# BLu85/AES-GCM-128-192-256-bits

Measured on NVIDIA B200. Metric: aes_gcm_enc_tag_throughput, higher is better.
Workload: dtype u8

## Files before the change

aes-gcm-128-192-256-bits_b200/csrc/capi.cu:

```cuda
#include <cuda.h>
#include <cuda_runtime.h>
#include <stdint.h>
#include <stdio.h>
#include <stdlib.h>
#include <string.h>
#include <new>
#include <vector>

#include "../../include/aesgcm_b200.h"
#include "kernels.h"
#include "host_sched.h"

namespace {

constexpr int kSlots = 3;
constexpr size_t kChunkBytesMax = 64u << 20;
constexpr size_t kMaxChunks = 8192;
constexpr uint64_t kAadInlineMax = 4096;
constexpr uint64_t kMaxBlocks = 0xFFFFFFFEull;

constexpr size_t SC_PART_CT = 0;
constexpr size_t SC_TAGCALC = 32;
constexpr size_t SC_OK = 48;
constexpr size_t SC_TAG = 64;
constexpr size_t SC_J0 = 80;
constexpr size_t SC_KEY = 96;
constexpr size_t SC_PARTS = 256;
constexpr size_t SC_PARTS_MAX = 1024;
constexpr size_t SC_BYTES = SC_PARTS + 16 * (SC_PARTS_MAX + 1);

template <class T>
struct GrownBuf {
    T* p = nullptr;
    size_t cap = 0;
};

struct PowCache {
    uint32_t* d = nullptr;
    uint64_t e = ~0ull;
    cudaEvent_t ev = nullptr;
    cudaStream_t st = nullptr;
};

}

struct agcm_ctx {
    int device = 0, sm_count = 0, ncta = 0, nt = 0;
    uint32_t* d_te0 = nullptr;
    KeyDev* d_key = nullptr;
    uint32_t* d_parts = nullptr;
    GrownBuf<uint32_t> seg_parts;
    uint8_t* d_scratch = nullptr;
    uint32_t* d_counters = nullptr;
    PowCache pow_n;
    PowCache pow_scale;
    uint32_t j0ctr = 1;
    GrownBuf<uint8_t> iv_stage;
    uint8_t** d_peer_bufs = nullptr;
    uint32_t* d_peer_status = nullptr;
    uint32_t* h_peer_status = nullptr;
    int peer_rank = 0, peer_world = 0;
    uint32_t peer_epoch = 0;
    uint64_t peer_timeout_ns = 10000000000ull;
    cudaStream_t peer_side = nullptr;
    cudaEvent_t peer_bulk_ev[AG_PEER_RING] = {};
    cudaEvent_t peer_fin_ev[AG_PEER_RING] = {};
    uint32_t h_rk[60];
    uint8_t h_H[16];
    uint8_t h_key_in[240];
    size_t key_in_len = 0;
    int key_in_mode = 0, key_in_pre = 0;
    int nr = 0;
    bool key_set = false;
    cudaError_t last_err = cudaSuccess;
    uint64_t launches = 0;
    bool timing = false;
    static constexpr int kTimingRing = 64;
    cudaEvent_t tev[2 * kTimingRing] = {};
    int tev_pending = 0;
    double t_total_ms = 0.0;
    uint64_t t_count = 0;
    cudaStream_t hs[kSlots] = {nullptr, nullptr, nullptr};
    uint8_t* d_stage[kSlots] = {nullptr, nullptr, nullptr};
    uint8_t* d_stage_aux[kSlots] = {nullptr, nullptr, nullptr};
    uint32_t* d_stage_parts[kSlots] = {nullptr, nullptr, nullptr};
    uint8_t* d_chunk_partials = nullptr;
    GrownBuf<uint8_t> aad_stage;
    uint32_t* d_tile_ticket = nullptr;
    bool no_ticket = false;
    GrownBuf<uint32_t> sort;
    void* tmap_encode = nullptr;
    GrownBuf<uint8_t> verify;
    bool pipeline_ready = false;
    size_t chunk_bytes = 32u << 20;
    size_t ramp_base = 1u << 20;
};

namespace {

int cuda_fail(agcm_ctx* c, cudaError_t e)
{
    if (c) c->last_err = e;
    return AGCM_E_CUDA;
}

#define AG_CUDA(ctx, call)                              \
    do {                                                \
        cudaError_t _e = (call);                        \
// ... 13 lines not shown
void iv_words(const uint8_t iv[12], uint32_t w[3])
{
    for (int i = 0; i < 3; ++i)
        w[i] = (uint32_t)iv[4 * i] | ((uint32_t)iv[4 * i + 1] << 8) | ((uint32_t)iv[4 * i + 2] << 16) |
               ((uint32_t)iv[4 * i + 3] << 24);
}

int timing_drain(agcm_ctx* c)
{
    for (int i = 0; i < c->tev_pending; ++i) {
        AG_CUDA(c, cudaEventSynchronize(c->tev[2 * i + 1]));
        float ms = 0.f;
        AG_CUDA(c, cudaEventElapsedTime(&ms, c->tev[2 * i], c->tev[2 * i + 1]));
        c->t_total_ms += ms;
        c->t_count++;
    }
    c->tev_pending = 0;
    return AGCM_OK;
}

template <class T>
int grow(agcm_ctx* c, GrownBuf<T>& b, size_t need)
{
    if (need <= b.cap) return AGCM_OK;
    AG_CUDA(c, cudaFree(b.p));
    b.p = nullptr;
    b.cap = 0;
    AG_CUDA(c, cudaMalloc(&b.p, need));
    b.cap = need;
    return AGCM_OK;
}

int zeroed_ticket(agcm_ctx* c, size_t words, cudaStream_t st, uint32_t*& ticket)
{
    if (!c->d_tile_ticket) AG_CUDA(c, cudaMalloc(&c->d_tile_ticket, 4 * sizeof(uint32_t)));
    AG_CUDA(c, cudaMemsetAsync(c->d_tile_ticket, 0, words * sizeof(uint32_t), st));
    ticket = c->d_tile_ticket;
    return AGCM_OK;
}

int pow_get(agcm_ctx* c, PowCache& pc, uint64_t e, cudaStream_t st)
{
    if (pc.ev && pc.st != st) AG_CUDA(c, cudaStreamWaitEvent(st, pc.ev, 0));
    if (pc.e == e) return AGCM_OK;
    AG_CUDA(c, ag_launch_pow(c->d_key, e, pc.d, st));
    c->launches++;
    pc.e = e;
    if (!pc.ev) AG_CUDA(c, cudaEventCreateWithFlags(&pc.ev, cudaEventDisableTiming));
    AG_CUDA(c, cudaEventRecord(pc.ev, st));
    pc.st = st;
    return AGCM_OK;
}

int peer_join_stream(agcm_ctx* c, cudaStream_t st)
{
    if (c->peer_epoch && c->peer_fin_ev[0]) AG_CUDA(c, cudaStreamWaitEvent(st, c->peer_fin_ev[c->peer_epoch % AG_PEER_RING], 0));
    return AGCM_OK;
}

int ensure_pow(agcm_ctx* c, uint64_t n_blocks, cudaStream_t st)
{
    if (c->pow_n.e != n_blocks) {
        int rc = peer_join_stream(c, st);
        if (rc) return rc;
    }
    return pow_get(c, c->pow_n, n_blocks, st);
}

FinishParams finish_params(const agcm_ctx* c, int decrypt, const uint8_t iv[12], const uint8_t* d_aad, uint64_t aad_len,
                           uint64_t ct_len, uint8_t* d_tag, uint8_t* d_ok, const uint32_t* hn)
{
    FinishParams f;
    memset(&f, 0, sizeof(f));
    memcpy(f.rk, c->h_rk, sizeof(f.rk));
    f.nr = (uint32_t)c->nr;
    iv_words(iv, f.iv);
    f.j0w = __builtin_bswap32(c->j0ctr);
    f.key = c->d_key;
    f.te0 = c->d_te0;
    f.aad = d_aad;
    f.aad_len = aad_len;
    f.ct_len = ct_len;
    f.tag_calc = decrypt ? c->d_scratch + SC_TAGCALC : d_tag;
    f.tag_expected = decrypt ? d_tag : nullptr;
    f.ok = decrypt ? d_ok : nullptr;
    f.hn = hn;
    return f;
}

int run_stream(agcm_ctx* c, int mode, const uint8_t iv[12], uint64_t first_block, const uint8_t* d_in, uint8_t* d_out,
               uint64_t n_bytes, uint64_t blocks_after, uint32_t* parts_raw, uint8_t* d_partial16, cudaStream_t st,
               uint32_t* counter, const FinishParams* ff = nullptr, uint32_t peer_epoch = 0, const uint8_t* gate = nullptr)
{
    if (n_bytes == 0) {
        if (d_partial16) AG_CUDA(c, cudaMemsetAsync(d_partial16, 0, 16, st));
        return AGCM_OK;
    }
    StreamParams p;
    memset(&p, 0, sizeof(p));
    memcpy(p.rk, c->h_rk, sizeof(p.rk));
    iv_words(iv, p.iv);
    p.ctr0 = (uint32_t)(c->j0ctr + 1 + first_block);
    p.j0w = __builtin_bswap32(c->j0ctr);
    p.n_bytes = n_bytes;
    p.in = d_in;
    p.out = d_out;
    p.key = c->d_key;
    p.te0 = c->d_te0;
    p.partials = parts_raw;
    p.gate = gate;
    if (mode != AG_MODE_CTR_ONLY) {
        p.done_counter = counter;
        p.scale_e = blocks_after;
        if (blocks_after && counter == c->d_counters && mode != AG_MODE_GHASH_ONLY) {
            if (!c->pow_scale.d) AG_CUDA(c, cudaMalloc(&c->pow_scale.d, 16));
            int rc = pow_get(c, c->pow_scale, blocks_after, st);
            if (rc) return rc;
            p.scale_pow = c->pow_scale.d;
        }
        p.out16 = d_partial16;
        if (ff) {
            p.fuse_finish = 1;
            p.aad = ff->aad;
            p.aad_len = ff->aad_len;
            p.ct_len = ff->ct_len;
            p.tag_calc = ff->tag_calc;
            p.tag_expected = ff->tag_expected;
            p.ok = ff->ok;
            p.hn = ff->hn;
        }
        if (peer_epoch) {
            p.peer_bufs = c->d_peer_bufs;
            p.peer_rank = (uint32_t)c->peer_rank;
            p.peer_world = (uint32_t)c->peer_world;
            p.peer_epoch = peer_epoch;
        }
    }
    cudaEvent_t ev0 = nullptr, ev1 = nullptr;
    if (c->timing) {
        if (c->tev_pending == agcm_ctx::kTimingRing) {
            int rc = timing_drain(c);
            if (rc) return rc;
        }
        ev0 = c->tev[2 * c->tev_pending];
        ev1 = c->tev[2 * c->tev_pending + 1];
        AG_CUDA(c, cudaEventRecord(ev0, st));
    }
    int ncta = c->ncta;
    const uint64_t blocks = (n_bytes + 15) >> 4;
    if (blocks <= (uint64_t)c->ncta * (uint64_t)c->nt) ncta = (int)((blocks + (uint64_t)c->nt - 1) / (uint64_t)c->nt);
    AG_CUDA(c, ag_launch_stream(p, c->nr, mode, ncta, c->nt, st));
    c->launches++;
    if (c->timing) {
        AG_CUDA(c, cudaEventRecord(ev1, st));
        c->tev_pending++;
    }
    return AGCM_OK;
}

int run_finish(agcm_ctx* c, int decrypt, const uint8_t iv[12], const uint8_t* d_parts16, int n_parts, const uint8_t* d_aad,
               uint64_t aad_len, uint64_t ct_len, uint8_t* d_tag, uint8_t* d_ok, cudaStream_t st)
{
    if (n_parts < 0 || (size_t)n_parts > SC_PARTS_MAX) return AGCM_E_BAD_ARG;
    if (decrypt && (!d_tag || !d_ok)) return AGCM_E_BAD_ARG;
    if (!decrypt && !d_tag) return AGCM_E_BAD_ARG;
    const uint64_t n_ct_blocks = (ct_len + 15) >> 4;
    if (n_ct_blocks > kMaxBlocks) return AGCM_E_COUNTER_OVERFLOW;
    const uint8_t* parts = d_parts16;
    int np = n_parts;
    const uint8_t* aad_inline = (aad_len && d_aad) ? d_aad : nullptr;
    if (aad_len && !d_aad) return AGCM_E_BAD_ARG;
    if (aad_len > kAadInlineMax) {
        uint8_t* list = c->d_scratch + SC_PARTS;
        if (n_parts) AG_CUDA(c, cudaMemcpyAsync(list, d_parts16, 16 * (size_t)n_parts, cudaMemcpyDeviceToDevice, st));
        int rc = run_stream(c, AG_MODE_GHASH_ONLY, iv, 0, d_aad, nullptr, aad_len, n_ct_blocks,
                            c->d_parts + 4 * AG_MAX_CTA, list + 16 * (size_t)n_parts, st, c->d_counters);
        if (rc) return rc;
        parts = list;
        np = n_parts + 1;
        aad_inline = nullptr;
    }
    if (aad_inline) {
        int rc = ensure_pow(c, n_ct_blocks, st);
        if (rc) return rc;
    }
    FinishParams f = finish_params(c, decrypt, iv, aad_inline, aad_len, ct_len, d_tag, d_ok, aad_inline ? c->pow_n.d : nullptr);
    f.parts = parts;
    f.n_parts = (uint32_t)np;
    AG_CUDA(c, ag_launch_finish(f, st));
    c->launches++;
    return AGCM_OK;
}

int derive_j0(agcm_ctx* c, const uint8_t* h_iv, size_t iv_len, uint8_t j0[16], cudaStream_t st)
{
    if (!h_iv || iv_len == 0 || iv_len > (1ull << 32)) return AGCM_E_BAD_LEN;
    if (!c->key_set) return AGCM_E_NO_KEY;
    const size_t padded = ((iv_len + 15) & ~(size_t)15) + 16;
    std::vector<uint8_t> buf(padded, 0);
    memcpy(buf.data(), h_iv, iv_len);
    const uint64_t bits = (uint64_t)iv_len * 8;
    for (int i = 0; i < 8; ++i) buf[padded - 1 - i] = (uint8_t)(bits >> (8 * i));
    int rc = grow(c, c->iv_stage, padded < 4096 ? 4096 : padded);
    if (rc) return rc;
    AG_CUDA(c, cudaMemcpyAsync(c->iv_stage.p, buf.data(), padded, cudaMemcpyHostToDevice, st));
    const uint8_t iv0[12] = {0};
    rc = run_stream(c, AG_MODE_GHASH_ONLY, iv0, 0, c->iv_stage.p, nullptr, padded, 0, c->d_parts, c->d_scratch + SC_J0, st,
                    c->d_counters);
// ... 172 lines not shown
    }
    if (e != cudaSuccess) {
        agcm_ctx_destroy(c);
        return AGCM_E_CUDA;
    }
    *out = c;
    return AGCM_OK;
}

int agcm_ctx_create(agcm_ctx** out, int device) { return agcm_ctx_create_ex(out, device, 0, 0); }

void agcm_ctx_destroy(agcm_ctx* c)
{
    if (!c) return;
    cudaSetDevice(c->device);
    cudaDeviceSynchronize();
    for (int s = 0; s < kSlots; ++s) {
        if (c->hs[s]) cudaStreamDestroy(c->hs[s]);
        cudaFree(c->d_stage[s]);
        cudaFree(c->d_stage_aux[s]);
        cudaFree(c->d_stage_parts[s]);
    }
    for (cudaEvent_t e : c->tev)
        if (e) cudaEventDestroy(e);
    if (c->d_key) cudaMemset(c->d_key, 0, sizeof(KeyDev));
    if (c->d_scratch) cudaMemset(c->d_scratch, 0, SC_BYTES);
    memset(c->h_rk, 0, sizeof(c->h_rk));
    memset(c->h_H, 0, sizeof(c->h_H));
    memset(c->h_key_in, 0, sizeof(c->h_key_in));
    cudaFree(c->d_chunk_partials);
    cudaFree(c->aad_stage.p);
    cudaFree(c->verify.p);
    cudaFree(c->d_tile_ticket);
    cudaFree(c->sort.p);
    cudaFree(c->d_te0);
    cudaFree(c->d_key);
    cudaFree(c->d_parts);
    cudaFree(c->seg_parts.p);
    cudaFree(c->iv_stage.p);
    cudaFree(c->d_scratch);
    cudaFree(c->d_counters);
    cudaFree(c->pow_n.d);
    cudaFree(c->pow_scale.d);
    cudaFree(c->d_peer_bufs);
    cudaFree(c->d_peer_status);
    if (c->h_peer_status) cudaFreeHost(c->h_peer_status);
    if (c->peer_side) cudaStreamDestroy(c->peer_side);
    for (uint32_t i = 0; i < AG_PEER_RING; ++i) {
        if (c->peer_bulk_ev[i]) cudaEventDestroy(c->peer_bulk_ev[i]);
        if (c->peer_fin_ev[i]) cudaEventDestroy(c->peer_fin_ev[i]);
    }
    if (c->pow_n.ev) cudaEventDestroy(c->pow_n.ev);
    if (c->pow_scale.ev) cudaEventDestroy(c->pow_scale.ev);
    delete c;
}

int agcm_last_cuda_error(const agcm_ctx* c) { return c ? (int)c->last_err : 0; }
const char* agcm_last_cuda_error_string(const agcm_ctx* c) { return cudaGetErrorString(c ? c->last_err : cudaSuccess); }
uint64_t agcm_launch_count(const agcm_ctx* c) { return c ? c->launches : 0; }

int agcm_timing_enable(agcm_ctx* c, int on)
{
    if (!c) return AGCM_E_BAD_ARG;
    AG_CUDA(c, cudaSetDevice(c->device));
    if (on && !c->tev[0])
        for (cudaEvent_t& e : c->tev) AG_CUDA(c, cudaEventCreate(&e));
    int rc = timing_drain(c);
    if (rc) return rc;
    c->timing = on != 0;
    c->t_total_ms = 0.0;
    c->t_count = 0;
    return AGCM_OK;
}

int agcm_timing_read(agcm_ctx* c, double* total_ms, uint64_t* n_launches)
{
    if (!c) return AGCM_E_BAD_ARG;
    int rc = timing_drain(c);
    if (rc) return rc;
    if (total_ms) *total_ms = c->t_total_ms;
    if (n_launches) *n_launches = c->t_count;
    return AGCM_OK;
}

int agcm_get_info(const agcm_ctx* c, int* n_cta, int* threads, int* sm_count)
{
    if (!c) return AGCM_E_BAD_ARG;
    if (n_cta) *n_cta = c->ncta;
    if (threads) *threads = c->nt;
    if (sm_count) *sm_count = c->sm_count;
    return AGCM_OK;
}

int agcm_key_expand(agcm_ctx* c, int mode, const uint8_t* d_keys, size_t n_keys, uint8_t* d_round_keys, void* stream)
{
    if (!c || (n_keys && (!d_keys || !d_round_keys))) return AGCM_E_BAD_ARG;
    if (!mode_to_nr(mode)) return AGCM_E_BAD_MODE;
    AG_CUDA(c, cudaSetDevice(c->device));
    AG_CUDA(c, ag_launch_key_expand(d_keys, n_keys, mode / 8, c->d_te0, d_round_keys, (cudaStream_t)stream));
    if (n_keys) c->launches++;
    return AGCM_OK;
}

int agcm_key_expand_host(agcm_ctx* c, int mode, const uint8_t* h_key, uint8_t* h_round_keys)
{
    if (!c || !h_key || !h_round_keys) return AGCM_E_BAD_ARG;
    const int nr = mode_to_nr(mode);
    if (!nr) return AGCM_E_BAD_MODE;
    AG_CUDA(c, cudaSetDevice(c->device));
    uint8_t* d_key = c->d_scratch + SC_KEY;
    uint8_t* d_rk = c->d_scratch + SC_PARTS;
    AG_CUDA(c, cudaMemcpy(d_key, h_key, (size_t)mode / 8, cudaMemcpyHostToDevice));
    AG_CUDA(c, ag_launch_key_expand(d_key, 1, mode / 8, c->d_te0, d_rk, nullptr));
    c->launches++;
    AG_CUDA(c, cudaMemcpy(h_round_keys, d_rk, (size_t)16 * (nr + 1), cudaMemcpyDeviceToHost));
    return AGCM_OK;
}

int agcm_set_key(agcm_ctx* c, int mode, int pre_expanded, const uint8_t* h_key, size_t key_len)
{
    if (!c || !h_key) return AGCM_E_BAD_ARG;
    const int nr = mode_to_nr(mode);
    if (!nr) return AGCM_E_BAD_MODE;
    const size_t want = pre_expanded ? (size_t)16 * (nr + 1) : (size_t)mode / 8;
    if (key_len != want) return AGCM_E_BAD_MODE;
    if (c->key_set && c->key_in_mode == mode && c->key_in_pre == (pre_expanded ? 1 : 0) && c->key_in_len == key_len &&
        memcmp(c->h_key_in, h_key, key_len) == 0)
        return AGCM_OK;
    AG_CUDA(c, cudaSetDevice(c->device));
    c->key_set = false;
    c->pow_n.e = ~0ull;
    c->pow_scale.e = ~0ull;
    KeyIn in;
    memset(&in, 0, sizeof(in));
    memcpy(in.w, h_key, key_len);
    in.key_bytes = (uint32_t)mode / 8;
    in.nr = (uint32_t)nr;
    in.pre_expanded = pre_expanded ? 1u : 0u;
    AG_CUDA(c, cudaDeviceSynchronize());
    AG_CUDA(c, ag_launch_key_setup(c->d_key, in, c->d_te0, c->nt, c->ncta, nullptr));
    c->launches++;
    static_assert(offsetof(KeyDev, rk) == 0 && offsetof(KeyDev, H) == 256, "KeyDev head layout");
    uint32_t head[68];
    AG_CUDA(c, cudaMemcpy(head, c->d_key, sizeof(head), cudaMemcpyDeviceToHost));
    memset(c->h_rk, 0, sizeof(c->h_rk));
    memcpy(c->h_rk, head, (size_t)16 * (nr + 1));
    const uint32_t* hw = head + 64;
    for (int i = 0; i < 4; ++i) {
        c->h_H[4 * i + 0] = (uint8_t)(hw[i] >> 24);
        c->h_H[4 * i + 1] = (uint8_t)(hw[i] >> 16);
        c->h_H[4 * i + 2] = (uint8_t)(hw[i] >> 8);
        c->h_H[4 * i + 3] = (uint8_t)hw[i];
    }
    c->nr = nr;
    memcpy(c->h_key_in, h_key, key_len);
    c->key_in_len = key_len;
    c->key_in_mode = mode;
    c->key_in_pre = pre_expanded ? 1 : 0;
    c->key_set = true;
    return AGCM_OK;
}

int agcm_get_round_keys(const agcm_ctx* c, uint8_t* h_round_keys, size_t cap)
{
    if (!c || !h_round_keys) return AGCM_E_BAD_ARG;
    if (!c->key_set) return AGCM_E_NO_KEY;
    const size_t n = (size_t)16 * (c->nr + 1);
    if (cap < n) return AGCM_E_BAD_LEN;
    memcpy(h_round_keys, c->h_rk, n);
    return (int)n;
}

int agcm_get_h(const agcm_ctx* c, uint8_t h_h16[16])
{
    if (!c || !h_h16) return AGCM_E_BAD_ARG;
    if (!c->key_set) return AGCM_E_NO_KEY;
    memcpy(h_h16, c->h_H, 16);
    return AGCM_OK;
}

int agcm_stream_part(agcm_ctx* c, int decrypt, const uint8_t h_iv12[12], uint64_t first_block, const uint8_t* d_in,
                     uint8_t* d_out, uint64_t n_bytes, uint64_t blocks_after, uint8_t* d_partial16, void* stream)
{
    if (!c || !h_iv12 || !d_partial16 || (n_bytes && (!d_in || !d_out))) return AGCM_E_BAD_ARG;
    if (!c->key_set) return AGCM_E_NO_KEY;
// ... 1133 lines not shown
```

aes-gcm-128-192-256-bits_b200/csrc/gcm_core.cuh:

```cuda
#pragma once
#include <stdint.h>
#include <string.h>
#include "aes_core.cuh"
#include "gf128.cuh"

enum : int {
    AG_MODE_ENC = 0,
    AG_MODE_DEC = 1,
    AG_MODE_GHASH_ONLY = 2,
    AG_MODE_CTR_ONLY = 3
};

constexpr int AG_MAX_CTA = 256;
#ifndef AG_NT_MAX
#define AG_NT_MAX 512
#endif
constexpr int AG_STREAM_NT_MAX = AG_NT_MAX;

struct KeyDev {
    uint32_t rk[60];
    uint32_t nr;
    uint32_t nt_stream;
    uint32_t ncta;
    uint32_t _pad;
    gf128 H;
    gf128 pow2[64];
    gf128 hpow_thread[AG_STREAM_NT_MAX + 1];
    gf128 hpow_cta[AG_MAX_CTA + 1];
    uint4 tab[8][256];
};

AG_HD void ag_load_block(const uint8_t* p, uint32_t nvalid, uint32_t x[4])
{
    if (nvalid == 16) {
#if defined(__CUDA_ARCH__)
        const uintptr_t a = (uintptr_t)p;
        if ((a & 15) == 0) {
            const uint4 v = *reinterpret_cast<const uint4*>(p);
            x[0] = v.x; x[1] = v.y; x[2] = v.z; x[3] = v.w;
            return;
        }
        if ((a & 3) == 0) {
            const uint32_t* q = reinterpret_cast<const uint32_t*>(p);
            x[0] = q[0]; x[1] = q[1]; x[2] = q[2]; x[3] = q[3];
            return;
        }
#endif
    }
    x[0] = x[1] = x[2] = x[3] = 0;
#pragma unroll
    for (uint32_t j = 0; j < 16; ++j)
        if (j < nvalid) x[j >> 2] |= (uint32_t)p[j] << (8 * (j & 3));
}

AG_HD void ag_store_block(uint8_t* p, uint32_t nvalid, const uint32_t x[4])
// ... 123 lines not shown
    bool have;
    __device__ __forceinline__ void init() { have = false; prev_addr = nullptr; prev = make_uint4(0, 0, 0, 0); }
    __device__ __forceinline__ void flush()
    {
        if (!have) return;
        const uint32_t ro = (uint32_t)((uintptr_t)prev_addr & 15);
        const uint32_t w[4] = {prev.x, prev.y, prev.z, prev.w};
        uint8_t* q = prev_addr + 16 - ro;
        for (uint32_t j = 16 - ro; j < 16; ++j) q[j - (16 - ro)] = (uint8_t)(w[j >> 2] >> (8 * (j & 3)));
        have = false;
    }
    __device__ __forceinline__ void put(uint8_t* q, const uint32_t o[4])
    {
        const uint32_t ro = (uint32_t)((uintptr_t)q & 15);
        const uint4 cur = make_uint4(o[0], o[1], o[2], o[3]);
        if (have && prev_addr + 16 == q) {
            *reinterpret_cast<uint4*>(q - ro) = ag_realign(prev, cur, 16 - ro);
        } else {
            flush();
            for (uint32_t j = 0; j < 16 - ro; ++j) q[j] = (uint8_t)(o[j >> 2] >> (8 * (j & 3)));
        }
        prev = cur;
        prev_addr = q;
        have = true;
    }
};
#endif

struct StreamParams {
    uint32_t rk[60];
    uint32_t iv[3];
    uint32_t ctr0;
    uint32_t j0w;
    uint64_t n_bytes;
    const uint8_t* in;
    uint8_t* out;
    const KeyDev* key;
    const uint32_t* te0;
    uint32_t* partials;
    uint32_t* done_counter;
    uint64_t scale_e;
    const uint32_t* scale_pow;
    uint8_t* out16;
    uint32_t fuse_finish;
    const uint8_t* aad;
    uint64_t aad_len, ct_len;
    uint8_t* tag_calc;
    const uint8_t* tag_expected;
    uint8_t* ok;
    const uint32_t* hn;
    uint8_t* const* peer_bufs;
    uint32_t peer_rank, peer_world, peer_epoch;
    const uint8_t* gate;
};

constexpr uint32_t AG_PEER_MAX = 16;
constexpr uint32_t AG_PEER_RING = 8;
constexpr uint32_t AG_PEER_AHEAD = 4;
constexpr uint32_t AG_PEER_FLAGS = AG_PEER_RING * AG_PEER_MAX * 16;
constexpr uint32_t AG_PEER_BYTES = AG_PEER_FLAGS + AG_PEER_RING * AG_PEER_MAX * 4;

#if defined(__CUDA_ARCH__)
__device__ __forceinline__ void ag_store_row_coop(uint8_t* dst, const uint32_t o[4], bool whole, uint32_t r)
{
    const uint32_t lane = threadIdx.x & 31;
    uint4 prev;
    prev.x = __shfl_up_sync(0xffffffffu, o[0], 1);
    prev.y = __shfl_up_sync(0xffffffffu, o[1], 1);
    prev.z = __shfl_up_sync(0xffffffffu, o[2], 1);
    prev.w = __shfl_up_sync(0xffffffffu, o[3], 1);
    const bool prev_whole = __shfl_up_sync(0xffffffffu, (int)whole, 1) != 0 && lane > 0;
    const bool next_whole = __shfl_down_sync(0xffffffffu, (int)whole, 1) != 0 && lane < 31;
    if (!whole) return;
    if (prev_whole) {
        *reinterpret_cast<uint4*>(dst - r) = ag_realign(prev, make_uint4(o[0], o[1], o[2], o[3]), 16 - r);
    } else {
        ag_store_block(dst, 16 - r, o);
    }
    if (!next_whole) {
        const uint4 t = ag_realign(make_uint4(o[0], o[1], o[2], o[3]), make_uint4(0, 0, 0, 0), 16 - r);
        const uint32_t tw[4] = {t.x, t.y, t.z, t.w};
        ag_store_block(dst + 16 - r, r, tw);
    }
}
#endif

template <int NR, int MODE, bool ALIGNED, class TE, class GH>
AG_HD gf128 ag_stream_lane(const StreamParams& p, uint32_t g, uint32_t Gt, TE&& te, GH&& gh)
{
    const uint32_t n_blocks = (uint32_t)((p.n_bytes + 15) >> 4);
    const uint32_t n_full = (uint32_t)(p.n_bytes >> 4);
    const uint32_t rows = (uint32_t)(((uint64_t)n_blocks + Gt - 1) / Gt);
    const uint32_t pad = (uint32_t)((uint64_t)rows * Gt - n_blocks);
    const uint32_t tail = (uint32_t)(p.n_bytes & 15);

    AesCtrConst cc;
    AesCtrCache cache;
    bool have = rows && g >= pad;
    uint32_t i = g - pad;
    if (MODE != AG_MODE_GHASH_ONLY) {
        cc = aes_ctr_precompute(p.rk, p.iv[0], p.iv[1], p.iv[2], te);
        aes_ctr_cache_fill(p.rk, cc, ag_bswap32(p.ctr0 + i) ^ p.rk[3], te, cache);
    }

    auto load = [&](uint32_t bi, uint32_t x[4]) {
        const uint8_t* src = p.in + 16 * (uint64_t)bi;
        if (ALIGNED && bi < n_full) {
#if defined(__CUDA_ARCH__)
            const uint4 v = *reinterpret_cast<const uint4*>(src);
            x[0] = v.x; x[1] = v.y; x[2] = v.z; x[3] = v.w;
#else
            ag_load_block(src, 16, x);
#endif
        } else {
            ag_load_block_in(src, bi < n_full ? 16u : tail, x, p.in, p.in + p.n_bytes);
        }
    };

    gf128 y = gf_zero();
    uint32_t xn[4] = {0, 0, 0, 0};
#if defined(__CUDA_ARCH__)
    const uint32_t r_out = (uint32_t)((uintptr_t)p.out & 15);
    const bool coop = !ALIGNED && MODE != AG_MODE_GHASH_ONLY && (r_out & 3) != 0;
#endif
    if (have) load(i, xn);
    for (uint32_t u = 0; u < rows; ++u) {
        uint32_t x[4] = {xn[0], xn[1], xn[2], xn[3]};
        if (u + 1 < rows) load(i + Gt, xn);
        if (MODE != AG_MODE_CTR_ONLY && u) y = gf_mul_table(y, gh);
        uint32_t o[4] = {0, 0, 0, 0};
        bool whole_out = false;
        if (have) {
            uint32_t s[4];
            if (MODE == AG_MODE_GHASH_ONLY) {
                s[0] = x[0]; s[1] = x[1]; s[2] = x[2]; s[3] = x[3];
            } else {
                uint32_t ks[4];
                aes_ctr_block_cached<NR>(p.rk, cc, cache, p.ctr0 + i, te, ks);
                o[0] = x[0] ^ ks[0]; o[1] = x[1] ^ ks[1]; o[2] = x[2] ^ ks[2]; o[3] = x[3] ^ ks[3];
                uint8_t* dst = p.out + 16 * (uint64_t)i;
                if (ALIGNED && i < n_full) {
#if defined(__CUDA_ARCH__)
                    *reinterpret_cast<uint4*>(dst) = make_uint4(o[0], o[1], o[2], o[3]);
#else
                    ag_store_block(dst, 16, o);
#endif
                } else {
                    const uint32_t nv = i < n_full ? 16u : tail;
#if defined(__CUDA_ARCH__)
                    if (coop && nv == 16) whole_out = true;
                    else
#endif
                        ag_store_block(dst, nv, o);
                    if (MODE == AG_MODE_ENC && nv != 16) ag_mask_block(o, nv);
                }
                if (MODE == AG_MODE_ENC) {
                    s[0] = o[0]; s[1] = o[1]; s[2] = o[2]; s[3] = o[3];
                } else {
                    s[0] = x[0]; s[1] = x[1]; s[2] = x[2]; s[3] = x[3];
                }
            }
            if (MODE != AG_MODE_CTR_ONLY) {
                y.w[0] ^= ag_bswap32(s[0]);
                y.w[1] ^= ag_bswap32(s[1]);
                y.w[2] ^= ag_bswap32(s[2]);
                y.w[3] ^= ag_bswap32(s[3]);
            }
        }
#if defined(__CUDA_ARCH__)
        if (coop) ag_store_row_coop(p.out + 16 * (uint64_t)i, o, whole_out, r_out);
#endif
        have = true;
        i += Gt;
    }
    return y;
}

struct BatchParams {
    uint32_t rk[60];
    const KeyDev* key;
    const uint32_t* te0;
    const uint8_t* keys;
    const uint8_t* iv;
    uint32_t iv_is_j0;
    const uint8_t* aad;
    const uint64_t* aad_off;
    const uint8_t* in;
    const uint64_t* in_off;
    uint8_t* out;
    uint8_t* tag;
    uint8_t* ok;
    uint64_t n_msgs;
    uint64_t len, stride, aad_len, aad_stride;
    const uint32_t* len_arr;
    const uint32_t* aad_len_arr;
    uint32_t split;
    uint32_t* seg_parts;
    uint32_t* ticket;
    const uint32_t* perm;
    const uint32_t* range;
    uint4* seg_acc;
    uint64_t* unit_desc;
    uint32_t* msg_acc;
    uint32_t* msg_cnt;
    uint32_t* msg_ej0;
    uint64_t quota_aad, quota_pt;
    uint64_t n_ids;
};

struct MsgDesc {
    const uint8_t* in;
    uint8_t* out;
    const uint8_t* aad;
    uint64_t len, aad_len;
    uint64_t total_len, total_aad_len;
    uint32_t ctr_off;
    uint32_t j0ctr;
    uint32_t last;
};

AG_HD MsgDesc ag_batch_msg(const BatchParams& p, uint64_t m)
{
    MsgDesc d;
    uint64_t o, l;
    if (p.in_off) { o = p.in_off[m]; l = p.in_off[m + 1] - o; }
    else { o = m * p.stride; l = p.len_arr ? (p.len_arr[m] < p.stride ? p.len_arr[m] : p.stride) : p.len; }
    d.in = p.in + o;
    d.out = p.out + o;
// ... 259 lines not shown
```

aes-gcm-128-192-256-bits_b200/csrc/kernels.cu:

```cuda
#include <cuda_runtime.h>
#include <stdint.h>
#include "gcm_core.cuh"
#include "kernels.h"
#include "smem_tables.cuh"

__global__ void k_key_expand(const uint8_t* __restrict__ keys, uint64_t n_keys, int key_bytes,
                             const uint32_t* __restrict__ te0, uint8_t* __restrict__ round_keys)
{
    __shared__ uint32_t sbox_s[256];
    for (int i = threadIdx.x; i < 256; i += blockDim.x) sbox_s[i] = (__ldg(te0 + i) >> 8) & 0xff;
    __syncthreads();
    const uint64_t i = (uint64_t)blockIdx.x * blockDim.x + threadIdx.x;
    if (i >= n_keys) return;
    uint8_t key[32];
    for (int j = 0; j < key_bytes; ++j) key[j] = keys[i * key_bytes + j];
    uint32_t rk[60];
    auto sb = [&](uint32_t b) { return sbox_s[b & 0xff]; };
    const int nr = aes_key_expand_words(key, key_bytes, sb, rk);
    uint32_t* dst = reinterpret_cast<uint32_t*>(round_keys + i * (uint64_t)(16 * (nr + 1)));
    for (int j = 0; j < 4 * (nr + 1); ++j) dst[j] = rk[j];
}

__global__ void __launch_bounds__(256) k_key_setup(KeyDev* kd, const __grid_constant__ KeyIn in,
                                                   const uint32_t* __restrict__ te0, uint32_t nt_stream, uint32_t ncta)
// ... 182 lines not shown
        const volatile uint32_t* f = reinterpret_cast<const volatile uint32_t*>(mine + AG_PEER_FLAGS + (slot * AG_PEER_MAX + w) * 4);
        uint64_t t0 = 0;
        uint32_t spins = 0;
        while (*f != p.epoch) {
            __nanosleep(64);
            if ((++spins & 255u) == 0) {
                uint64_t now;
                asm volatile("mov.u64 %0, %%globaltimer;" : "=l"(now));
                if (!t0) t0 = now;
                else if (now - t0 > p.timeout_ns) { arrived = false; break; }
            }
        }
    }
    __threadfence_system();
    gf128 t = gf_zero();
    if (w < p.world) {
        const uint4 q = __ldcv(reinterpret_cast<const uint4*>(mine + (slot * AG_PEER_MAX + w) * 16));
        t.w[0] = q.x; t.w[1] = q.y; t.w[2] = q.z; t.w[3] = q.w;
    }
    const gf128 s = warp_xor(t);
    if (!__all_sync(0xffffffffu, arrived)) {
        if (w == 0) {
            const uint32_t z[4] = {0, 0, 0, 0};
            ag_store_block(p.f.tag_calc, 16, z);
            if (p.f.ok) *p.f.ok = 0;
            if (p.status_dev) *p.status_dev = 1;
            if (p.status_host) *p.status_host = 1;
            __threadfence_system();
        }
        return;
    }
    FinishArgs a{p.f.rk, p.f.nr, p.f.iv, p.f.j0w, p.f.key, p.f.te0, p.f.aad, p.f.aad_len, p.f.ct_len, p.f.tag_calc,
                 p.f.tag_expected, p.f.ok, p.f.hn, false};
    finish_warp(a, s);
}

__global__ void __launch_bounds__(32) k_stream_finish(const __grid_constant__ FinishParams p)
{
    const uint32_t lane = threadIdx.x;
    gf128 s = gf_zero();
    for (uint32_t j = lane; j < p.n_parts; j += 32) {
        uint32_t x[4];
        ag_load_block(p.parts + 16 * j, 16, x);
        s = gf_xor(s, gf_from_le_words(x[0], x[1], x[2], x[3]));
    }
    s = warp_xor(s);
    FinishArgs a{p.rk, p.nr, p.iv, p.j0w, p.key, p.te0, p.aad, p.aad_len, p.ct_len, p.tag_calc, p.tag_expected, p.ok, p.hn, false};
    finish_warp(a, s);
}

template <int NR, int MODE, bool ALIGNED>
__global__ void __launch_bounds__(AG_STREAM_NT_MAX, 1) k_stream(const __grid_constant__ StreamParams p)
{
    const uint32_t tid = threadIdx.x, lane = tid & 31, nt = blockDim.x;
    if (MODE == AG_MODE_CTR_ONLY && p.gate && __ldcg(p.gate) == 0) return;
    if (MODE != AG_MODE_GHASH_ONLY) stage_te0(p.te0);
    if (MODE != AG_MODE_CTR_ONLY) fill_gh_tables(p.key->tab[7], nullptr);
    __syncthreads();
    if (MODE != AG_MODE_GHASH_ONLY) expand_aes_tables();
    __syncthreads();

    TeSmem te{ag_smem, lane * 4};
    GhSmem gh{ag_smem + SM_GH, (lane & 7) * 16};
    const uint32_t Gt = gridDim.x * nt;
    const uint32_t g = blockIdx.x * nt + tid;
    gf128 y = ag_stream_lane<NR, MODE, ALIGNED>(p, g, Gt, te, gh);
    if (MODE == AG_MODE_CTR_ONLY) return;

    gf128 w_cta = gf_zero();
    if (tid == 0) w_cta = p.key->hpow_cta[gridDim.x - 1 - blockIdx.x];
    if (__any_sync(0xffffffffu, (y.w[0] | y.w[1] | y.w[2] | y.w[3]) != 0)) y = gf_mul(y, p.key->hpow_thread[nt - tid]);
    y = warp_xor(y);
    gf128* red = reinterpret_cast<gf128*>(ag_smem + SM_MISC);
    if (lane == 0) red[tid >> 5] = y;
    __syncthreads();
    if (tid < 32) {
        gf128 v = (tid < (nt >> 5)) ? red[tid] : gf_zero();
        v = warp_xor(v);
        if (tid == 0) {
            v = gf_mul(v, w_cta);
            uint32_t* dst = p.partials + 4 * blockIdx.x;
            dst[0] = v.w[0]; dst[1] = v.w[1]; dst[2] = v.w[2]; dst[3] = v.w[3];
        }
        uint32_t ticket = 0;
        if (p.done_counter) {
            if (tid == 0) {
                __threadfence();
                ticket = atomicAdd(p.done_counter, 1u);
            }
            ticket = __shfl_sync(0xffffffffu, ticket, 0);
            if (ticket == gridDim.x - 1) {
                __threadfence();
                gf128 s = gf_zero();
                for (uint32_t j = tid; j < gridDim.x; j += 32) {
                    const uint4 q = __ldcg(reinterpret_cast<const uint4*>(p.partials) + j);
                    s.w[0] ^= q.x; s.w[1] ^= q.y; s.w[2] ^= q.z; s.w[3] ^= q.w;
                }
                s = warp_xor(s);
                if (p.scale_e) {
                    gf128 he;
                    if (p.scale_pow) {
                        he.w[0] = __ldcg(p.scale_pow + 0); he.w[1] = __ldcg(p.scale_pow + 1);
                        he.w[2] = __ldcg(p.scale_pow + 2); he.w[3] = __ldcg(p.scale_pow + 3);
                    } else {
                        he = warp_gf_pow(p.key, p.scale_e);
                    }
                    s = gf_mul(s, he);
                }
                if (p.out16 && tid == 0) {
                    const uint32_t o[4] = {ag_bswap32(s.w[0]), ag_bswap32(s.w[1]), ag_bswap32(s.w[2]), ag_bswap32(s.w[3])};
                    ag_store_block(p.out16, 16, o);
                }
                if (p.peer_world) ag_peer_post(p.peer_bufs, p.peer_rank, p.peer_world, p.peer_epoch, s);
                if (p.fuse_finish) {
                    FinishArgs a{p.rk, (uint32_t)NR, p.iv, p.j0w, p.key, p.te0, p.aad, p.aad_len, p.ct_len, p.tag_calc,
                                 p.tag_expected, p.ok, p.hn, MODE != AG_MODE_GHASH_ONLY};
                    finish_warp(a, s);
                }
                if (tid == 0) *p.done_counter = 0;
            }
        }
    }
}

__global__ void __launch_bounds__(32) k_pow(const KeyDev* kd, uint64_t e, uint32_t* __restrict__ out)
{
    const gf128 r = warp_gf_pow(kd, e);
    if (threadIdx.x == 0) { out[0] = r.w[0]; out[1] = r.w[1]; out[2] = r.w[2]; out[3] = r.w[3]; }
}

__global__ void __launch_bounds__(32) k_xor_parts(const uint8_t* __restrict__ parts, uint32_t n, uint8_t* __restrict__ out)
{
    const uint32_t lane = threadIdx.x;
    gf128 s = gf_zero();
    for (uint32_t j = lane; j < n; j += 32) {
        uint32_t x[4];
        ag_load_block(parts + 16 * j, 16, x);
        s.w[0] ^= x[0]; s.w[1] ^= x[1]; s.w[2] ^= x[2]; s.w[3] ^= x[3];
    }
    s = warp_xor(s);
    if (lane == 0) ag_store_block(out, 16, s.w);
}


size_t ag_smem_bytes() { return kSmemBytes; }

template <int NR, int MODE>
static cudaError_t launch_stream_t(const StreamParams& p, int ncta, int nt, cudaStream_t st)
{
    const bool aligned = (((uintptr_t)p.in | (uintptr_t)p.out) & 15) == 0;
    cudaError_t e;
    if (aligned) {
        e = cudaFuncSetAttribute(k_stream<NR, MODE, true>, cudaFuncAttributeMaxDynamicSharedMemorySize, (int)kSmemBytes);
        if (e != cudaSuccess) return e;
        k_stream<NR, MODE, true><<<ncta, nt, kSmemBytes, st>>>(p);
    } else {
        e = cudaFuncSetAttribute(k_stream<NR, MODE, false>, cudaFuncAttributeMaxDynamicSharedMemorySize, (int)kSmemBytes);
        if (e != cudaSuccess) return e;
        k_stream<NR, MODE, false><<<ncta, nt, kSmemBytes, st>>>(p);
    }
    return cudaGetLastError();
}

template <int NR>
static cudaError_t launch_stream_nr(const StreamParams& p, int mode, int ncta, int nt, cudaStream_t st)
{
    switch (mode) {
        case AG_MODE_ENC: return launch_stream_t<NR, AG_MODE_ENC>(p, ncta, nt, st);
        case AG_MODE_DEC: return launch_stream_t<NR, AG_MODE_DEC>(p, ncta, nt, st);
        case AG_MODE_GHASH_ONLY: return launch_stream_t<NR, AG_MODE_GHASH_ONLY>(p, ncta, nt, st);
        case AG_MODE_CTR_ONLY: return launch_stream_t<NR, AG_MODE_CTR_ONLY>(p, ncta, nt, st);
    }
    return cudaErrorInvalidValue;
}

cudaError_t ag_launch_stream(const StreamParams& p, int nr, int mode, int ncta, int nt, cudaStream_t st)
{
    switch (nr) {
        case 10: return launch_stream_nr<10>(p, mode, ncta, nt, st);
        case 12: return launch_stream_nr<12>(p, mode, ncta, nt, st);
        case 14: return launch_stream_nr<14>(p, mode, ncta, nt, st);
    }
    return cudaErrorInvalidValue;
}

cudaError_t ag_launch_key_expand(const uint8_t* keys, uint64_t n_keys, int key_bytes, const uint32_t* te0,
                                 uint8_t* round_keys, cudaStream_t st)
{
    if (n_keys == 0) return cudaSuccess;
    const int nt = 128;
    const uint64_t nb = (n_keys + nt - 1) / nt;
    k_key_expand<<<(unsigned)nb, nt, 0, st>>>(keys, n_keys, key_bytes, te0, round_keys);
    return cudaGetLastError();
}

cudaError_t ag_launch_key_setup(KeyDev* kd, const KeyIn& in, const uint32_t* te0, int nt_stream, int ncta,
                                cudaStream_t st)
{
    k_key_setup<<<1, 256, 0, st>>>(kd, in, te0, (uint32_t)nt_stream, (uint32_t)ncta);
    return cudaGetLastError();
}

cudaError_t ag_launch_pow(const KeyDev* kd, uint64_t e, uint32_t* out, cudaStream_t st)
{
    k_pow<<<1, 32, 0, st>>>(kd, e, out);
    return cudaGetLastError();
}

cudaError_t ag_launch_xor_parts(const uint8_t* parts, uint32_t n, uint8_t* out, cudaStream_t st)
{
    k_xor_parts<<<1, 32, 0, st>>>(parts, n, out);
    return cudaGetLastError();
}

cudaError_t ag_preload_peer_kernels()
{
    cudaFuncAttributes a;
    cudaError_t e = cudaFuncGetAttributes(&a, k_peer_post);
    if (e == cudaSuccess) e = cudaFuncGetAttributes(&a, k_peer_finish);
    if (e == cudaSuccess) e = cudaFuncGetAttributes(&a, k_pow);
    if (e == cudaSuccess) e = cudaFuncGetAttributes(&a, k_xor_parts);
    return e;
}

cudaError_t ag_launch_peer_finish(const PeerFinishParams& p, cudaStream_t st)
{
    k_peer_finish<<<1, 32, 0, st>>>(p);
    return cudaGetLastError();
}

cudaError_t ag_launch_peer_post(uint8_t* const* peer_bufs, uint32_t rank, uint32_t world, uint32_t epoch,
                                const uint8_t* partial16, cudaStream_t st)
{
    k_peer_post<<<1, 32, 0, st>>>(peer_bufs, rank, world, epoch, partial16);
    return cudaGetLastError();
}

cudaError_t ag_launch_finish(const FinishParams& p, cudaStream_t st)
{
    k_stream_finish<<<1, 32, 0, st>>>(p);
    return cudaGetLastError();
}
```

aes-gcm-128-192-256-bits_b200/csrc/kernels.h:

```cpp
#pragma once
#include <cuda.h>
#include <cuda_runtime.h>
#include <stdint.h>
#include "gcm_core.cuh"

struct FinishParams {
    uint32_t rk[60];
    uint32_t nr;
    uint32_t iv[3];
    uint32_t j0w;
    const KeyDev* key;
    const uint32_t* te0;
    const uint8_t* parts;
    uint32_t n_parts;
    const uint8_t* aad;
    uint64_t aad_len;
    uint64_t ct_len;
    uint8_t* tag_calc;
    const uint8_t* tag_expected;
    uint8_t* ok;
    const uint32_t* hn;
};

struct PeerFinishParams {
    FinishParams f;
    uint8_t* const* peer_bufs;
    uint32_t rank, world, epoch;
    uint64_t timeout_ns;
    uint32_t* status_dev;
    volatile uint32_t* status_host;
};

cudaError_t ag_launch_stream(const StreamParams& p, int nr, int mode, int ncta, int nt, cudaStream_t st);
cudaError_t ag_launch_batch(const BatchParams& p, int nr, int decrypt, int g, int ncta, int nt, cudaStream_t st);
struct TileParams {
    BatchParams b;
    CUtensorMap tm_in, tm_out;
    CUtensorMap tm_aad;
    uint32_t aad_tiled;
    uint32_t* ticket;
};
constexpr uint32_t AG_TILE_BOX_BYTES = 32, AG_TILE_BOX_MSGS = 32;
cudaError_t ag_launch_batch_tile(const TileParams& p, int nr, int decrypt, int gather, int ncta, cudaStream_t st);
cudaError_t ag_launch_batch_perkey_tile(const TileParams& p, int nr, int decrypt, int max_cta, cudaStream_t st);
cudaError_t ag_launch_batch_warp(const BatchParams& p, int nr, int decrypt, int ncta, cudaStream_t st);
cudaError_t ag_launch_len_sort(const BatchParams& p, uint32_t* hist4096, uint32_t* ranges6, uint32_t* perm, cudaStream_t st);
cudaError_t ag_launch_batch_cta(const BatchParams& p, int nr, int decrypt, int ncta, int nt, cudaStream_t st);
cudaError_t ag_launch_batch_perkey(const BatchParams& p, int nr, int decrypt, int max_cta, cudaStream_t st);
cudaError_t ag_launch_batch_verify(const BatchParams& p, int nr, int g, int ncta, int nt, cudaStream_t st);
cudaError_t ag_launch_batch_warp_verify(const BatchParams& p, int nr, int ncta, cudaStream_t st);
cudaError_t ag_launch_batch_ctr_gated(const BatchParams& p, int nr, uint64_t n_slots, uint64_t bpr, int max_cta, cudaStream_t st);
cudaError_t ag_launch_key_expand(const uint8_t* keys, uint64_t n_keys, int key_bytes, const uint32_t* te0,
                                 uint8_t* round_keys, cudaStream_t st);
struct KeyIn {
    uint32_t w[60];
    uint32_t key_bytes;
    uint32_t nr;
    uint32_t pre_expanded;
};
cudaError_t ag_launch_key_setup(KeyDev* kd, const KeyIn& in, const uint32_t* te0, int nt_stream, int ncta,
                                cudaStream_t st);
cudaError_t ag_launch_pow(const KeyDev* kd, uint64_t e, uint32_t* out4, cudaStream_t st);
cudaError_t ag_launch_finish(const FinishParams& p, cudaStream_t st);
cudaError_t ag_launch_peer_finish(const PeerFinishParams& p, cudaStream_t st);
cudaError_t ag_preload_peer_kernels();
cudaError_t ag_launch_peer_post(uint8_t* const* peer_bufs, uint32_t rank, uint32_t world, uint32_t epoch,
                                const uint8_t* partial16, cudaStream_t st);
cudaError_t ag_launch_batch_j0(const KeyDev* kd, const uint8_t* iv, const uint64_t* iv_off, uint64_t iv_len, uint64_t n,
                               uint8_t* j0, cudaStream_t st);
cudaError_t ag_launch_xor_parts(const uint8_t* parts16, uint32_t n, uint8_t* out16, cudaStream_t st);
size_t ag_smem_bytes();
```

Before: 514.8.

## Give each lane contiguous spans of blocks in the stream kernel with per-launch GHASH weights

Block indices are now assigned in spans of eight consecutive blocks per warp sub-group instead of a grid-wide stride. This gives each lane sequential counters, which lets it use a sequential AES counter cache, and lets stores coalesce within runs. GHASH then steps by H^8 instead of the H power tied to the grid width, so the per-thread and per-CTA weight powers depend on the row count. A new small kernel computes these weights and caches them per counter slot. This adds an extra launch whenever the length or CTA count changes, plus event-based stream ordering.

After: 517.5 (median of 6 runs). No clear change (+0.5%).

```diff
diff --git a/aes-gcm-128-192-256-bits_b200/csrc/capi.cu b/aes-gcm-128-192-256-bits_b200/csrc/capi.cu
--- a/aes-gcm-128-192-256-bits_b200/csrc/capi.cu
+++ b/aes-gcm-128-192-256-bits_b200/csrc/capi.cu
@@ -38,6 +38,14 @@
 struct PowCache {
     uint32_t* d = nullptr;
     uint64_t e = ~0ull;
+    cudaEvent_t ev = nullptr;
+    cudaStream_t st = nullptr;
+};
+
+struct SpanWeights {
+    gf128* d = nullptr;
+    uint32_t rows = 0;
+    int ncta = 0;
     cudaEvent_t ev = nullptr;
     cudaStream_t st = nullptr;
 };
@@ -54,6 +62,7 @@
     uint32_t* d_counters = nullptr;
     PowCache pow_n;
     PowCache pow_scale;
+    SpanWeights span_w[1 + kSlots];
     uint32_t j0ctr = 1;
     GrownBuf<uint8_t> iv_stage;
     uint8_t** d_peer_bufs = nullptr;
@@ -173,6 +182,19 @@
     return AGCM_OK;
 }
 
+int span_weights(agcm_ctx* c, SpanWeights& w, uint32_t rows, int ncta, cudaStream_t st)
+{
+    if (!w.d) AG_CUDA(c, cudaMalloc(&w.d, sizeof(gf128) * (AG_STREAM_NT_MAX + AG_MAX_CTA)));
+    if (!w.ev) AG_CUDA(c, cudaEventCreateWithFlags(&w.ev, cudaEventDisableTiming));
+    if (w.st && w.st != st) AG_CUDA(c, cudaStreamWaitEvent(st, w.ev, 0));
+    if (w.rows == rows && w.ncta == ncta) return AGCM_OK;
+    AG_CUDA(c, ag_launch_span_weights(c->d_key, rows, c->nt, ncta, w.d, st));
+    c->launches++;
+    w.rows = rows;
+    w.ncta = ncta;
+    return AGCM_OK;
+}
+
 int peer_join_stream(agcm_ctx* c, cudaStream_t st)
 {
     if (c->peer_epoch && c->peer_fin_ev[0]) AG_CUDA(c, cudaStreamWaitEvent(st, c->peer_fin_ev[c->peer_epoch % AG_PEER_RING], 0));
@@ -257,6 +279,20 @@
             p.peer_epoch = peer_epoch;
         }
     }
+    int ncta = c->ncta;
+    const uint64_t blocks = (n_bytes + 15) >> 4;
+    if (blocks <= (uint64_t)c->ncta * (uint64_t)c->nt) ncta = (int)((blocks + (uint64_t)c->nt - 1) / (uint64_t)c->nt);
+    const uint32_t rows = ag_stream_rows(n_bytes, (uint32_t)(ncta * c->nt));
+    SpanWeights* sw = nullptr;
+    const bool aligned = (((uintptr_t)d_in | (uintptr_t)d_out) & 15) == 0;
+    if ((mode == AG_MODE_ENC || mode == AG_MODE_DEC) && aligned && rows > 1) {
+        const ptrdiff_t k = counter - c->d_counters;
+        if (!counter || k < 0 || k > kSlots) return AGCM_E_BAD_ARG;
+        sw = &c->span_w[k];
+        int rc = span_weights(c, *sw, rows, ncta, st);
+        if (rc) return rc;
+        p.span_w = sw->d;
+    }
     cudaEvent_t ev0 = nullptr, ev1 = nullptr;
     if (c->timing) {
         if (c->tev_pending == agcm_ctx::kTimingRing) {
@@ -267,14 +303,15 @@
         ev1 = c->tev[2 * c->tev_pending + 1];
         AG_CUDA(c, cudaEventRecord(ev0, st));
     }
-    int ncta = c->ncta;
-    const uint64_t blocks = (n_bytes + 15) >> 4;
-    if (blocks <= (uint64_t)c->ncta * (uint64_t)c->nt) ncta = (int)((blocks + (uint64_t)c->nt - 1) / (uint64_t)c->nt);
     AG_CUDA(c, ag_launch_stream(p, c->nr, mode, ncta, c->nt, st));
     c->launches++;
     if (c->timing) {
         AG_CUDA(c, cudaEventRecord(ev1, st));
         c->tev_pending++;
+    }
+    if (sw) {
+        AG_CUDA(c, cudaEventRecord(sw->ev, st));
+        sw->st = st;
     }
     return AGCM_OK;
 }
@@ -553,6 +590,10 @@
     }
     if (c->pow_n.ev) cudaEventDestroy(c->pow_n.ev);
     if (c->pow_scale.ev) cudaEventDestroy(c->pow_scale.ev);
+    for (SpanWeights& w : c->span_w) {
+        cudaFree(w.d);
+        if (w.ev) cudaEventDestroy(w.ev);
+    }
     delete c;
 }
 
@@ -632,6 +673,7 @@
     c->key_set = false;
     c->pow_n.e = ~0ull;
     c->pow_scale.e = ~0ull;
+    for (SpanWeights& w : c->span_w) w.rows = 0;
     KeyIn in;
     memset(&in, 0, sizeof(in));
     memcpy(in.w, h_key, key_len);
diff --git a/aes-gcm-128-192-256-bits_b200/csrc/gcm_core.cuh b/aes-gcm-128-192-256-bits_b200/csrc/gcm_core.cuh
--- a/aes-gcm-128-192-256-bits_b200/csrc/gcm_core.cuh
+++ b/aes-gcm-128-192-256-bits_b200/csrc/gcm_core.cuh
@@ -1,6 +1,7 @@
 #pragma once
 #include <stdint.h>
 #include <string.h>
+#include <type_traits>
 #include "aes_core.cuh"
 #include "gf128.cuh"
 
@@ -230,6 +231,7 @@
     uint8_t* const* peer_bufs;
     uint32_t peer_rank, peer_world, peer_epoch;
     const uint8_t* gate;
+    const gf128* span_w;
 };
 
 constexpr uint32_t AG_PEER_MAX = 16;
@@ -239,16 +241,16 @@
 constexpr uint32_t AG_PEER_BYTES = AG_PEER_FLAGS + AG_PEER_RING * AG_PEER_MAX * 4;
 
 #if defined(__CUDA_ARCH__)
-__device__ __forceinline__ void ag_store_row_coop(uint8_t* dst, const uint32_t o[4], bool whole, uint32_t r)
-{
-    const uint32_t lane = threadIdx.x & 31;
+__device__ __forceinline__ void ag_store_row_coop(uint8_t* dst, const uint32_t o[4], bool whole, uint32_t r, uint32_t run)
+{
+    const uint32_t lane = threadIdx.x & 31, in_run = lane & (run - 1);
     uint4 prev;
     prev.x = __shfl_up_sync(0xffffffffu, o[0], 1);
     prev.y = __shfl_up_sync(0xffffffffu, o[1], 1);
     prev.z = __shfl_up_sync(0xffffffffu, o[2], 1);
     prev.w = __shfl_up_sync(0xffffffffu, o[3], 1);
-    const bool prev_whole = __shfl_up_sync(0xffffffffu, (int)whole, 1) != 0 && lane > 0;
-    const bool next_whole = __shfl_down_sync(0xffffffffu, (int)whole, 1) != 0 && lane < 31;
+    const bool prev_whole = __shfl_up_sync(0xffffffffu, (int)whole, 1) != 0 && in_run > 0;
+    const bool next_whole = __shfl_down_sync(0xffffffffu, (int)whole, 1) != 0 && in_run < run - 1;
     if (!whole) return;
     if (prev_whole) {
         *reinterpret_cast<uint4*>(dst - r) = ag_realign(prev, make_uint4(o[0], o[1], o[2], o[3]), 16 - r);
@@ -263,22 +265,50 @@
 }
 #endif
 
-template <int NR, int MODE, bool ALIGNED, class TE, class GH>
-AG_HD gf128 ag_stream_lane(const StreamParams& p, uint32_t g, uint32_t Gt, TE&& te, GH&& gh)
+constexpr uint32_t AG_SPAN = 8;
+
+AG_HD uint32_t ag_stream_rows(uint64_t n_bytes, uint32_t Gt)
+{
+    return (uint32_t)((((n_bytes + 15) >> 4) + Gt - 1) / Gt);
+}
+
+AG_HD uint64_t ag_span_lane_exp(uint32_t tid, uint32_t nt, uint32_t rows, uint32_t W)
+{
+    return (uint64_t)rows * (nt - W - W * (tid / W)) + (W - tid % W);
+}
+AG_HD uint64_t ag_span_cta_exp(uint32_t cta, uint32_t ncta, uint32_t nt, uint32_t rows)
+{
+    return (uint64_t)rows * nt * (ncta - 1 - cta);
+}
+
+template <int NR, int MODE, bool ALIGNED, bool SPAN, class TE, class GH>
+AG_HD gf128 ag_stream_lane(const StreamParams& p, uint32_t g, uint32_t Gt, uint32_t W, TE&& te, GH&& gh)
 {
     const uint32_t n_blocks = (uint32_t)((p.n_bytes + 15) >> 4);
     const uint32_t n_full = (uint32_t)(p.n_bytes >> 4);
-    const uint32_t rows = (uint32_t)(((uint64_t)n_blocks + Gt - 1) / Gt);
+    const uint32_t rows = ag_stream_rows(p.n_bytes, Gt);
     const uint32_t pad = (uint32_t)((uint64_t)rows * Gt - n_blocks);
     const uint32_t tail = (uint32_t)(p.n_bytes & 15);
 
+    uint32_t i, step, u0;
+    if (SPAN) {
+        const uint64_t s0 = (uint64_t)W * rows * (g / W) + g % W;
+        step = W;
+        u0 = s0 >= pad ? 0u : (uint32_t)((pad - s0 + W - 1) / W);
+        i = (uint32_t)(s0 - pad);
+    } else {
+        step = Gt;
+        u0 = g >= pad ? 0u : 1u;
+        i = g - pad;
+    }
+    bool have = rows && u0 == 0;
+
     AesCtrConst cc;
-    AesCtrCache cache;
-    bool have = rows && g >= pad;
-    uint32_t i = g - pad;
+    typename std::conditional<SPAN, AesCtrSeqCache, AesCtrCache>::type cache;
+    cache.key = 0xFFFFFFFFu;
     if (MODE != AG_MODE_GHASH_ONLY) {
         cc = aes_ctr_precompute(p.rk, p.iv[0], p.iv[1], p.iv[2], te);
-        aes_ctr_cache_fill(p.rk, cc, ag_bswap32(p.ctr0 + i) ^ p.rk[3], te, cache);
+        if constexpr (!SPAN) aes_ctr_cache_fill(p.rk, cc, ag_bswap32(p.ctr0 + i) ^ p.rk[3], te, cache);
     }
 
     auto load = [&](uint32_t bi, uint32_t x[4]) {
@@ -304,7 +334,7 @@
     if (have) load(i, xn);
     for (uint32_t u = 0; u < rows; ++u) {
         uint32_t x[4] = {xn[0], xn[1], xn[2], xn[3]};
-        if (u + 1 < rows) load(i + Gt, xn);
+        if (u + 1 < rows && u + 1 >= u0) load(i + step, xn);
         if (MODE != AG_MODE_CTR_ONLY && u) y = gf_mul_table(y, gh);
         uint32_t o[4] = {0, 0, 0, 0};
         bool whole_out = false;
@@ -314,7 +344,7 @@
                 s[0] = x[0]; s[1] = x[1]; s[2] = x[2]; s[3] = x[3];
             } else {
                 uint32_t ks[4];
-                aes_ctr_block_cached<NR>(p.rk, cc, cache, p.ctr0 + i, te, ks);
+                aes_ctr_block_auto<NR>(p.rk, cc, cache, p.ctr0 + i, te, ks);
                 o[0] = x[0] ^ ks[0]; o[1] = x[1] ^ ks[1]; o[2] = x[2] ^ ks[2]; o[3] = x[3] ^ ks[3];
                 uint8_t* dst = p.out + 16 * (uint64_t)i;
                 if (ALIGNED && i < n_full) {
@@ -346,12 +376,18 @@
             }
         }
 #if defined(__CUDA_ARCH__)
-        if (coop) ag_store_row_coop(p.out + 16 * (uint64_t)i, o, whole_out, r_out);
-#endif
-        have = true;
-        i += Gt;
+        if (coop) ag_store_row_coop(p.out + 16 * (uint64_t)i, o, whole_out, r_out, SPAN ? W : 32u);
+#endif
+        have = u + 1 >= u0;
+        i += step;
     }
     return y;
+}
+
+template <int NR, int MODE, bool ALIGNED, class TE, class GH>
+AG_HD gf128 ag_stream_lane(const StreamParams& p, uint32_t g, uint32_t Gt, TE&& te, GH&& gh)
+{
+    return ag_stream_lane<NR, MODE, ALIGNED, false>(p, g, Gt, 1u, te, gh);
 }
 
 struct BatchParams {
diff --git a/aes-gcm-128-192-256-bits_b200/csrc/kernels.cu b/aes-gcm-128-192-256-bits_b200/csrc/kernels.cu
--- a/aes-gcm-128-192-256-bits_b200/csrc/kernels.cu
+++ b/aes-gcm-128-192-256-bits_b200/csrc/kernels.cu
@@ -258,10 +258,11 @@
 template <int NR, int MODE, bool ALIGNED>
 __global__ void __launch_bounds__(AG_STREAM_NT_MAX, 1) k_stream(const __grid_constant__ StreamParams p)
 {
+    constexpr bool SPAN = ALIGNED && MODE != AG_MODE_GHASH_ONLY;
     const uint32_t tid = threadIdx.x, lane = tid & 31, nt = blockDim.x;
     if (MODE == AG_MODE_CTR_ONLY && p.gate && __ldcg(p.gate) == 0) return;
     if (MODE != AG_MODE_GHASH_ONLY) stage_te0(p.te0);
-    if (MODE != AG_MODE_CTR_ONLY) fill_gh_tables(p.key->tab[7], nullptr);
+    if (MODE != AG_MODE_CTR_ONLY) fill_gh_tables(SPAN ? p.key->tab[3] : p.key->tab[7], nullptr);
     __syncthreads();
     if (MODE != AG_MODE_GHASH_ONLY) expand_aes_tables();
     __syncthreads();
@@ -270,12 +271,14 @@
     GhSmem gh{ag_smem + SM_GH, (lane & 7) * 16};
     const uint32_t Gt = gridDim.x * nt;
     const uint32_t g = blockIdx.x * nt + tid;
-    gf128 y = ag_stream_lane<NR, MODE, ALIGNED>(p, g, Gt, te, gh);
+    gf128 y = ag_stream_lane<NR, MODE, ALIGNED, SPAN>(p, g, Gt, AG_SPAN, te, gh);
     if (MODE == AG_MODE_CTR_ONLY) return;
 
+    const bool per_launch = SPAN && p.span_w;
     gf128 w_cta = gf_zero();
-    if (tid == 0) w_cta = p.key->hpow_cta[gridDim.x - 1 - blockIdx.x];
-    if (__any_sync(0xffffffffu, (y.w[0] | y.w[1] | y.w[2] | y.w[3]) != 0)) y = gf_mul(y, p.key->hpow_thread[nt - tid]);
+    if (tid == 0) w_cta = per_launch ? p.span_w[nt + blockIdx.x] : p.key->hpow_cta[gridDim.x - 1 - blockIdx.x];
+    if (__any_sync(0xffffffffu, (y.w[0] | y.w[1] | y.w[2] | y.w[3]) != 0))
+        y = gf_mul(y, per_launch ? p.span_w[tid] : p.key->hpow_thread[nt - tid]);
     y = warp_xor(y);
     gf128* red = reinterpret_cast<gf128*>(ag_smem + SM_MISC);
     if (lane == 0) red[tid >> 5] = y;
@@ -335,6 +338,16 @@
     if (threadIdx.x == 0) { out[0] = r.w[0]; out[1] = r.w[1]; out[2] = r.w[2]; out[3] = r.w[3]; }
 }
 
+__global__ void __launch_bounds__(256) k_span_weights(const KeyDev* kd, uint32_t rows, uint32_t nt, uint32_t ncta,
+                                                      gf128* __restrict__ out)
+{
+    const uint32_t w = (blockIdx.x * blockDim.x + threadIdx.x) >> 5;
+    if (w >= nt + ncta) return;
+    const uint64_t e = w < nt ? ag_span_lane_exp(w, nt, rows, AG_SPAN) : ag_span_cta_exp(w - nt, ncta, nt, rows);
+    const gf128 r = warp_gf_pow(kd, e);
+    if ((threadIdx.x & 31) == 0) out[w] = r;
+}
+
 __global__ void __launch_bounds__(32) k_xor_parts(const uint8_t* __restrict__ parts, uint32_t n, uint8_t* __restrict__ out)
 {
     const uint32_t lane = threadIdx.x;
@@ -413,6 +426,13 @@
     return cudaGetLastError();
 }
 
+cudaError_t ag_launch_span_weights(const KeyDev* kd, uint32_t rows, int nt, int ncta, gf128* out, cudaStream_t st)
+{
+    const int warps = nt + ncta;
+    k_span_weights<<<(warps + 7) / 8, 256, 0, st>>>(kd, rows, (uint32_t)nt, (uint32_t)ncta, out);
+    return cudaGetLastError();
+}
+
 cudaError_t ag_launch_xor_parts(const uint8_t* parts, uint32_t n, uint8_t* out, cudaStream_t st)
 {
     k_xor_parts<<<1, 32, 0, st>>>(parts, n, out);
diff --git a/aes-gcm-128-192-256-bits_b200/csrc/kernels.h b/aes-gcm-128-192-256-bits_b200/csrc/kernels.h
--- a/aes-gcm-128-192-256-bits_b200/csrc/kernels.h
+++ b/aes-gcm-128-192-256-bits_b200/csrc/kernels.h
@@ -61,6 +61,7 @@
 cudaError_t ag_launch_key_setup(KeyDev* kd, const KeyIn& in, const uint32_t* te0, int nt_stream, int ncta,
                                 cudaStream_t st);
 cudaError_t ag_launch_pow(const KeyDev* kd, uint64_t e, uint32_t* out4, cudaStream_t st);
+cudaError_t ag_launch_span_weights(const KeyDev* kd, uint32_t rows, int nt, int ncta, gf128* out, cudaStream_t st);
 cudaError_t ag_launch_finish(const FinishParams& p, cudaStream_t st);
 cudaError_t ag_launch_peer_finish(const PeerFinishParams& p, cudaStream_t st);
 cudaError_t ag_preload_peer_kernels();
```
